# tsurumeso/vocal-remover

Measured on NVIDIA H100. Metric: seconds-of-audio/sec separated (n_fft=2048, hop=1024), higher is better.
Workload: dtype bf16x3 (split-bf16 operands hi+lo, 3 wgmma passes, fp32 accumulate); fft/lstm fp32

## Files before the change

### vocal-remover_b200/build.py

```python
import os
import subprocess
import sys
from concurrent.futures import ThreadPoolExecutor

HERE = os.path.dirname(os.path.abspath(__file__))
CSRC = os.path.join(HERE, 'csrc')
OBJ = os.path.join(HERE, 'build')
LIB = os.path.join(HERE, 'libvr_b200.so')
SOURCES = ['api.cu', 'engine.cu', 'conv_simt.cu', 'conv_tc.cu', 'conv_tc_rows.cu', 'conv_tc_halo.cu', 'elementwise.cu', 'lstm.cu', 'fft.cu', 'resample.cu', 'flac.cu', 'flac_encode.cu', 'bsseval.cu', 'wiener.cu']
NVCC = os.environ.get('NVCC', '/usr/local/cuda/bin/nvcc')
FLAGS = ['-gencode', 'arch=compute_90a,code=sm_90a', '-O3', '-lineinfo', '-std=c++17',
         '-Xcompiler', '-fPIC', '-Xcompiler', '-fvisibility=hidden', '--expt-relaxed-constexpr']


def _newest_header():
    hs = [os.path.join(CSRC, f) for f in os.listdir(CSRC) if f.endswith(('.h', '.cuh'))]
    hs.append(os.path.join(HERE, '..', 'include', 'vr_b200.h'))
    return max(os.path.getmtime(h) for h in hs)


def build(verbose=False, force=False):
    global OBJ, LIB
    extra = os.environ.get('VR_BUILD_FLAGS', '').split()
    if os.environ.get('VR_BUILD_TAG'):
        OBJ = os.path.join(HERE, 'build_' + os.environ['VR_BUILD_TAG'])
        LIB = os.path.join(HERE, 'libvr_b200_%s.so' % os.environ['VR_BUILD_TAG'])
    os.makedirs(OBJ, exist_ok=True)
    hdr = _newest_header()
    jobs = []
    for src in SOURCES:
        s = os.path.join(CSRC, src)
        o = os.path.join(OBJ, src.replace('.cu', '.o'))
        if force or not os.path.exists(o) or os.path.getmtime(o) < max(os.path.getmtime(s), hdr):
            jobs.append((s, o))

    def cc(job):
        s, o = job
        cmd = [NVCC] + FLAGS + extra + ['-c', s, '-o', o]
        if verbose:
            cmd += ['-Xptxas', '-v']
        r = subprocess.run(cmd, capture_output=True, text=True)
        if r.returncode != 0:
            raise RuntimeError('nvcc failed for %s:\n%s\n%s' % (s, r.stdout, r.stderr))
        return r.stderr

    with ThreadPoolExecutor(max_workers=min(8, max(1, len(jobs)))) as ex:
        logs = list(ex.map(cc, jobs))
    if verbose:
        for lg in logs:
            print(lg)
    objs = [os.path.join(OBJ, s.replace('.cu', '.o')) for s in SOURCES]
    if jobs or not os.path.exists(LIB):
        cmd = [NVCC, '-shared', '-o', LIB] + objs + ['-gencode', 'arch=compute_90a,code=sm_90a']
        r = subprocess.run(cmd, capture_output=True, text=True)
        if r.returncode != 0:
            raise RuntimeError('link failed:\n%s\n%s' % (r.stdout, r.stderr))
    return LIB


if __name__ == '__main__':
    print(build(verbose='-v' in sys.argv, force='-f' in sys.argv))
```

### vocal-remover_b200/csrc/api.cu

```cuda
#include <stdio.h>
#include <string.h>

#include <string>

#include "../../include/vr_b200.h"
#include "engine.h"
#include "kernels.h"
#include "tc_plan.h"

struct vr_ctx {
  vr::Engine* eng;
  std::string err;
};

static std::string g_create_err;

static int fail(vr_ctx* c, const std::string& m) {
  (c ? c->err : g_create_err) = m;
  return -1;
}
static void use_device(const vr_ctx* c) {
  if (c && c->eng) cudaSetDevice(c->eng->cfg().device);
}
static int done(vr_ctx* c, bool ok) {
// ... 339 lines not shown
  return 0;
}

int64_t vr_launch_count(const vr_ctx* ctx) { return ctx && ctx->eng ? ctx->eng->launches : 0; }

int vr_profile_enable(vr_ctx* ctx, int32_t on) {
  CHECK_CTX(ctx);
  ctx->eng->profile_enable(on != 0);
  return 0;
}

int vr_profile_read(vr_ctx* ctx, double* out6) {
  CHECK_CTX(ctx);
  return done(ctx, ctx->eng->profile_read(out6));
}

int vr_profile_dump(vr_ctx* ctx, char* text, int64_t cap, int64_t* needed) {
  CHECK_CTX(ctx);
  std::string t;
  if (!ctx->eng->profile_dump(t)) return done(ctx, false);
  if (needed) *needed = (int64_t)t.size() + 1;
  if (text && cap > 0) {
    const size_t n = t.size() < (size_t)cap - 1 ? t.size() : (size_t)cap - 1;
    memcpy(text, t.data(), n);
    text[n] = 0;
  }
  return 0;
}

int vr_debug_conv(vr_ctx* ctx, const float* x, int32_t N, int32_t Cin, int32_t H, int32_t W, const float* w,
                  const float* bias, int32_t Cout, int32_t k, int32_t stride, int32_t dil_h, int32_t dil_w, int32_t act,
                  int32_t use_tc, float* y, void* stream) {
  CHECK_CTX(ctx);
  return done(ctx, ctx->eng->debug_conv(x, N, Cin, H, W, w, bias, Cout, k, stride, dil_h, dil_w, act, use_tc, y,
                                        (cudaStream_t)stream));
}

int vr_debug_decoder(vr_ctx* ctx, const float* low, int32_t N, int32_t Cl, int32_t h, int32_t w, const float* skip,
                     int32_t Cs, const float* wgt, const float* bias, int32_t Cout, int32_t act, int32_t fused, float* y,
                     void* stream) {
  CHECK_CTX(ctx);
  return done(ctx, ctx->eng->debug_decoder(low, N, Cl, h, w, skip, Cs, wgt, bias, Cout, act, fused, y,
                                           (cudaStream_t)stream));
}

int vr_debug_tensor(vr_ctx* ctx, const char* name, int32_t n0, int32_t n, float* out, int64_t* shape4, void* stream) {
  CHECK_NET(ctx);
  if (!name || !shape4) return fail(ctx, "vr_debug_tensor: name and shape4 are required");
  return done(ctx, ctx->eng->debug_tensor(name, n0, n, out, shape4, (cudaStream_t)stream));
}

int vr_debug_set(int32_t key, int32_t value) {
  int* knob = key == 0 ? &vr::g_debug.trace : key == 2 ? &vr::g_debug.rows_wide : key == 3 ? &vr::g_debug.halo
            : key == 6 ? &vr::g_debug.kskip : key == 7 ? &vr::g_debug.crop_mask : nullptr;
  if (!knob) return -1;
  *knob = value;
  return 0;
}

int64_t vr_debug_trace(uint64_t* host_out, int64_t capacity) {
  return vr::tc_rows_read_trace((unsigned long long*)host_out, (long long)capacity);
}

}
```

### vocal-remover_b200/csrc/conv_tc.cu

```cuda
#include <cuda.h>
#include <stdio.h>

#include <map>
#include <tuple>

#include "engine.h"
#include "tc_common.cuh"
#include "tc_plan.h"

namespace vr {

static constexpr int kMaxStages = 8;
static constexpr int kConsumerWarps = 8;
static constexpr int kThreads = 32 * kConsumerWarps + 32;
static constexpr int kStaticSmem = 2048;

struct TcParams {
  int N, Ho, Wo, Wt, Ht, Nt, tiles_w, tiles_h, m_tiles, n_tiles;
  int stride, pad_h, pad_w, dil_h, dil_w, KW;
  int cchunks, total_sub, CinPadTC, Cout, act, stages;
  bf16* out_hi;
  bf16* out_lo;
  int64_t osn, osh;
  int osw;
// ... 103 lines not shown
        held.release(ring, lane);
        held.hold(ring);
        ring.advance();
      }
      wg_wait<0>();
      held.release_last(ring, lane);

      const int nt = tile % p.n_tiles;
      const int mt = tile / p.n_tiles;
      const int w0 = (mt % p.tiles_w) * p.Wt;
      const int h0 = ((mt / p.tiles_w) % p.tiles_h) * p.Ht;
      const int n0 = (mt / (p.tiles_w * p.tiles_h)) * p.Nt;
      const int c_lane = nt * BN + 2 * (lane & 3);
#pragma unroll
      for (int hr = 0; hr < 2; ++hr) {
        const int row = 64 * wg + 16 * (warp & 3) + (lane >> 2) + 8 * hr;
        const int dw = row % p.Wt;
        const int dh = (row / p.Wt) % p.Ht;
        const int n = n0 + row / (p.Wt * p.Ht);
        if (n >= p.N) continue;
        const int64_t obase = (int64_t)n * p.osn + (int64_t)(h0 + dh) * p.osh + (int64_t)(w0 + dw) * p.osw;
#pragma unroll
        for (int j = 0; j < BN / 8; ++j)
          epilogue_pair(acc[4 * j + 2 * hr], acc[4 * j + 2 * hr + 1], bias_s, c_lane + 8 * j, p.Cout, slope,
                        p.out_hi + obase, p.out_lo + obase);
      }
    }
  }
}

#define VR_TC_FOR_BN(X, KB) X(KB, 16) X(KB, 32) X(KB, 48) X(KB, 64) X(KB, 80) X(KB, 96) X(KB, 112) X(KB, 128)
#define VR_TC_FOR_ALL(X) VR_TC_FOR_BN(X, 64) VR_TC_FOR_BN(X, 32) VR_TC_FOR_BN(X, 16)


TcDebug g_debug;

static constexpr int kMaxDevices = 64;
const TcDevice& tc_device() {
  static TcDevice table[kMaxDevices];
  static TcDevice none;
  int dev = -1;
  if (cudaGetDevice(&dev) != cudaSuccess || dev < 0 || dev >= kMaxDevices) return none;
  TcDevice& d = table[dev];
  if (!d.ok) {
    if (cudaDeviceGetAttribute(&d.max_smem, cudaDevAttrMaxSharedMemoryPerBlockOptin, dev) != cudaSuccess ||
        cudaDeviceGetAttribute(&d.num_sms, cudaDevAttrMultiProcessorCount, dev) != cudaSuccess)
      return none;
#define VR_TC_SET_SMEM(KB, BN) \
  cudaFuncSetAttribute(conv_tc_kernel<KB, BN>, cudaFuncAttributeMaxDynamicSharedMemorySize, d.max_smem - kStaticSmem);
    VR_TC_FOR_ALL(VR_TC_SET_SMEM)
#undef VR_TC_SET_SMEM
    tc_rows_set_attributes(d.max_smem);
    tc_halo_set_attributes(d.max_smem);
    d.ok = true;
  }
  return d;
}

typedef CUresult (*EncodeTiledFn)(CUtensorMap*, CUtensorMapDataType, cuuint32_t, void*, const cuuint64_t*,
                                  const cuuint64_t*, const cuuint32_t*, const cuuint32_t*, CUtensorMapInterleave,
                                  CUtensorMapSwizzle, CUtensorMapL2promotion, CUtensorMapFloatOOBfill);
static EncodeTiledFn tc_encode_fn() {
  static EncodeTiledFn fn = nullptr;
  if (!fn) {
    void* p = nullptr;
    cudaDriverEntryPointQueryResult q;
    if (cudaGetDriverEntryPoint("cuTensorMapEncodeTiled", &p, cudaEnableDefault, &q) == cudaSuccess &&
        q == cudaDriverEntryPointSuccess)
      fn = (EncodeTiledFn)p;
  }
  return fn;
}

static CUtensorMapSwizzle swizzle_for(int KB) {
  return KB == 64 ? CU_TENSOR_MAP_SWIZZLE_128B : KB == 32 ? CU_TENSOR_MAP_SWIZZLE_64B : CU_TENSOR_MAP_SWIZZLE_32B;
}

static uint16_t tc_f2bf(float f) {
  uint32_t u;
  memcpy(&u, &f, 4);
  if ((u & 0x7fffffffu) > 0x7f800000u) return (uint16_t)((u >> 16) | 0x40);
  uint32_t r = 0x7fffu + ((u >> 16) & 1u);
  return (uint16_t)((u + r) >> 16);
}
static float tc_bf2f(uint16_t h) {
  uint32_t u = (uint32_t)h << 16;
  float f;
  memcpy(&f, &u, 4);
  return f;
}

struct TileGeom {
  int Wt, Ht, Nt;
  bool ok;
};
static TileGeom tile_geom(int Ho, int Wo) {
  TileGeom g{0, 0, 0, false};
  if (Wo <= 0 || Ho <= 0) return g;
  if (Wo >= 128) {
    if (Wo % 128) return g;
    g.Wt = 128; g.Ht = 1; g.Nt = 1;
  } else {
    if (128 % Wo) return g;
    g.Wt = Wo;
    g.Ht = 128 / Wo < Ho ? 128 / Wo : Ho;
    if (Ho % g.Ht) return g;
    if ((128 / Wo) % g.Ht) return g;
    g.Nt = 128 / (g.Wt * g.Ht);
  }
  g.ok = true;
  return g;
}

struct NTiling {
  int BN, n_tiles;
};
static NTiling n_tiling(const ConvLayer& L, bool rows, bool rows_wide) {
  const int cout16 = round_up(L.Cout, 16);
  if (rows) {
    const int BN = cout16 == 16 ? 16 : (rows_wide && cout16 % 64 == 0 ? 64 : 32);
    return {BN, ceil_div(cout16, BN)};
  }
  const int n_tiles = ceil_div(cout16, 128);
  return {round_up(ceil_div(cout16, n_tiles), 16), n_tiles};
}

TcKind tc_choose(const ConvLayer& L, int H, int W, bool rows_wide) {
  if (!(L.k == 1 || L.k == 3) || !(L.stride == 1 || L.stride == 2) || L.Cout < 4) return TC_NONE;
  const TileGeom g = tile_geom(H, W);
  if (!g.ok || g.Wt * L.stride > 256 || g.Ht * L.stride > 256) return TC_NONE;
  const bool k3s1 = L.k == 3 && L.stride == 1 && L.dil_h == 1 && L.dil_w == 1;
  const NTiling r = n_tiling(L, true, rows_wide), t = n_tiling(L, false, false);
  if (k3s1 && W % 128 == 0 && H % 8 == 0 && tc_rows_has(r.BN) && r.n_tiles * r.BN <= 256) return TC_ROWS;
  if (k3s1 && (W == 16 || W == 32 || W == 64) && H % (128 / W) == 0 && tc_halo_has(t.BN) &&
      t.n_tiles * t.BN <= 256 && g_debug.halo != 1)
    return TC_HALO;
  if (t.n_tiles * t.BN > 256) return TC_NONE;
  return TC_GENERIC;
}

template <class At>
static std::vector<uint16_t> split_bf16(const ConvLayer& L, const float* wp, int rows, int K, At at) {
  std::vector<uint16_t> planes((size_t)2 * rows * K, 0);
  const size_t lo = (size_t)rows * K;
  for (int co = 0; co < L.Cout; ++co)
    for (int t = 0; t < L.k * L.k; ++t)
      for (int ci = 0; ci < L.CinPad; ++ci) {
        const float w = wp[((size_t)t * L.CinPad + ci) * L.CoutPad + co];
        const uint16_t hi = tc_f2bf(w);
        const size_t i = at(co, t, ci);
        planes[i] = hi;
        planes[lo + i] = tc_f2bf(w - tc_bf2f(hi));
      }
  return planes;
}

static unsigned long long weight_group_mask(const ConvLayer& L, const float* wp, int CinPad) {
  if (CinPad / 8 > 64) return ~0ull;
  unsigned long long m = 0x3ull;
  for (int ci = 0; ci < L.CinPad; ++ci) {
    bool any = false;
    for (int t = 0; t < L.k * L.k && !any; ++t)
      for (int co = 0; co < L.Cout && !any; ++co) any = wp[((size_t)t * L.CinPad + ci) * L.CoutPad + co] != 0.f;
    if (any) m |= 1ull << (ci / 8);
  }
  return m;
}

static bool encode_weight_map(TcConv& tc, int rows, int K, int box_rows, std::string& err, const std::string& name) {
  cuuint64_t dims[3] = {(cuuint64_t)K, (cuuint64_t)rows, 2};
  cuuint64_t strides[2] = {(cuuint64_t)K * 2, (cuuint64_t)rows * K * 2};
  cuuint32_t box[3] = {(cuuint32_t)tc.KB, (cuuint32_t)box_rows, 2};
  cuuint32_t es[3] = {1, 1, 1};
  CUresult r = tc_encode_fn()(&tc.map_b, CU_TENSOR_MAP_DATA_TYPE_BFLOAT16, 3, tc.w_planes.get(), dims, strides, box, es,
                              CU_TENSOR_MAP_INTERLEAVE_NONE, swizzle_for(tc.KB), CU_TENSOR_MAP_L2_PROMOTION_L2_256B,
                              CU_TENSOR_MAP_FLOAT_OOB_FILL_NONE);
  if (r != CUDA_SUCCESS) {
    err = "cuTensorMapEncodeTiled(weights) failed for " + name + " code " + std::to_string((int)r);
    return false;
  }
  return true;
}

const CUtensorMap* tc_activation_map(TcConv& tc, const ActView& v, int bw, int bh, int bn, int es, std::string& err,
                                     const std::string& name) {
  const ViewKey key = std::make_tuple((const void*)v.hi, (const void*)v.lo, v.N, v.H, v.W, v.C, bw, bh, bn);
  auto it = tc.map_a.find(key);
  if (it != tc.map_a.end()) return &it->second;
  const int64_t plane = (const char*)v.lo - (const char*)v.hi;
  if (v.sw % 8 || v.sh % 8 || v.sn % 8 || (reinterpret_cast<uintptr_t>(v.hi) & 15) || plane <= 0 || plane % 16) {
    err = "internal: the input of " + name + " is not 16-byte aligned or its lo plane does not follow its hi plane";
    return nullptr;
  }
  cuuint64_t dims[5] = {(cuuint64_t)v.C, (cuuint64_t)v.W, (cuuint64_t)v.H, (cuuint64_t)v.N, 2};
  cuuint64_t strides[4] = {(cuuint64_t)v.sw * 2, (cuuint64_t)v.sh * 2, (cuuint64_t)v.sn * 2, (cuuint64_t)plane};
  cuuint32_t box[5] = {(cuuint32_t)tc.KB, (cuuint32_t)bw, (cuuint32_t)bh, (cuuint32_t)bn, 2};
  cuuint32_t estr[5] = {1, (cuuint32_t)es, (cuuint32_t)es, 1, 1};
  CUtensorMap m;
  CUresult r = tc_encode_fn()(&m, CU_TENSOR_MAP_DATA_TYPE_BFLOAT16, 5, (void*)v.hi, dims, strides, box, estr,
                              CU_TENSOR_MAP_INTERLEAVE_NONE, swizzle_for(tc.KB), CU_TENSOR_MAP_L2_PROMOTION_L2_256B,
                              CU_TENSOR_MAP_FLOAT_OOB_FILL_NONE);
  if (r != CUDA_SUCCESS) {
    err = "cuTensorMapEncodeTiled(activations) failed for " + name + " code " + std::to_string((int)r);
    return nullptr;
  }
  return &tc.map_a.emplace(key, m).first->second;
}

bool tc_prepare(ConvLayer& L, const float* w, const float* b, int H, int W, bool rows_wide, std::string& err) {
  const TcKind kind = tc_choose(L, H, W, rows_wide);
  if (kind == TC_NONE) return true;
  if (!tc_encode_fn()) {
    err = "cuTensorMapEncodeTiled is not available from the driver";
    return false;
  }
  auto tc = std::make_shared<TcConv>();
  tc->kind = kind;
  tc->H = H; tc->W = W;
  const NTiling nt = n_tiling(L, kind == TC_ROWS, rows_wide);
  const int BN = nt.BN, cin16 = round_up(L.CinPad, 16);
  tc->BN = BN; tc->n_tiles = nt.n_tiles;
  tc->KB = kind != TC_GENERIC ? 32 : cin16 % 64 == 0 ? 64 : cin16 % 32 == 0 ? 32 : 16;
  const int CinPad = round_up(L.CinPad, tc->KB);
  tc->CinPad = CinPad;
  tc->chunks = CinPad / tc->KB;
  tc->kmask = weight_group_mask(L, w, CinPad);
  const int rows = nt.n_tiles * BN;
  std::vector<uint16_t> planes;
  int brows, K;
  if (kind == TC_ROWS) {
    brows = 3 * rows;
    K = 3 * CinPad;
    planes = split_bf16(L, w, brows, K, [&](int co, int t, int ci) {
      return (size_t)(co / BN * 3 * BN + (2 - t / 3) * BN + co % BN) * K + (size_t)(t % 3) * CinPad + ci;
    });
  } else {
    brows = rows;
    K = L.k * L.k * CinPad;
    planes = split_bf16(L, w, brows, K, [&](int co, int t, int ci) { return (size_t)co * K + (size_t)t * CinPad + ci; });
  }
  std::vector<float> bias((size_t)rows, 0.f);
  for (int co = 0; co < L.Cout; ++co) bias[(size_t)co] = b[co];
  if (tc->w_planes.alloc(planes.size() * 2) != cudaSuccess || tc->bias.alloc(bias.size() * 4) != cudaSuccess) {
    err = "cudaMalloc failed while packing tensor-core weights for " + L.name;
    return false;
  }
  if (!upload(tc->w_planes.get(), planes.data(), planes.size() * 2, err) ||
      !upload(tc->bias.get(), bias.data(), bias.size() * 4, err) ||
      !encode_weight_map(*tc, brows, K, kind == TC_ROWS ? 3 * BN : BN, err, L.name))
    return false;
  L.tc = tc;
  return true;
}

cudaError_t tc_launch(const ConvLayer& L, const ActView& in, const ActView& out, cudaStream_t s, std::string& err,
                      const ConvFusion& f) {
  TcConv& tc = *L.tc;
  if (out.H != tc.H || out.W != tc.W || (in.H - 1) / L.stride + 1 != out.H || (in.W - 1) / L.stride + 1 != out.W) {
    err = "internal: " + L.name + " is launched on maps of another size than it was prepared for";
    return cudaErrorInvalidValue;
  }
  if (tc.kind == TC_ROWS) return tc_rows_launch(L, tc, in, out, s, err, f);
  if (!f.empty()) {
    err = "tc_launch: fused work is only implemented in the row-streaming kernel";
    return cudaErrorInvalidValue;
  }
  if (tc.kind == TC_HALO) return tc_halo_launch(L, tc, in, out, s, err);
  const TileGeom g = tile_geom(out.H, out.W);
  const CUtensorMap* map_a = tc_activation_map(tc, in, g.Wt * L.stride, g.Ht * L.stride, g.Nt, L.stride, err, L.name);
  if (!map_a) return cudaErrorInvalidValue;
  const int SUBS = 64 / tc.KB;
  TcParams p;
  p.N = out.N; p.Ho = out.H; p.Wo = out.W;
  p.Wt = g.Wt; p.Ht = g.Ht; p.Nt = g.Nt;
  p.tiles_w = out.W / g.Wt; p.tiles_h = out.H / g.Ht;
  p.m_tiles = p.tiles_w * p.tiles_h * ceil_div(out.N, g.Nt);
  p.n_tiles = tc.n_tiles;
  p.stride = L.stride; p.dil_h = L.dil_h; p.dil_w = L.dil_w;
  p.pad_h = L.dil_h * (L.k / 2); p.pad_w = L.dil_w * (L.k / 2);
  p.KW = L.k;
  p.cchunks = tc.chunks; p.total_sub = L.k * L.k * tc.chunks;
  p.CinPadTC = tc.CinPad; p.Cout = L.Cout; p.act = L.act;
  const int stage_bytes = SUBS * (2 * 128 * tc.KB * 2 + 2 * tc.BN * tc.KB * 2);
  const TcDevice& dv = tc_device();
  if (!dv.ok) {
    err = "tc_launch: cannot query the current device";
    return cudaErrorInvalidValue;
  }
  const int dyn = dv.max_smem - kStaticSmem;
  p.stages = (dyn - 1024) / stage_bytes;
  if (p.stages > kMaxStages) p.stages = kMaxStages;
  if (p.stages < 2) {
    err = "tc_launch: shared memory too small for two pipeline stages";
    return cudaErrorInvalidValue;
  }
  p.out_hi = out.hi; p.out_lo = out.lo;
  p.osn = out.sn; p.osh = out.sh; p.osw = out.sw;
  p.bias = tc.bias.get();
  const int total_tiles = p.m_tiles * p.n_tiles;
  const int grid = total_tiles < dv.num_sms ? total_tiles : dv.num_sms;
#define VR_TC_LAUNCH(KB_, BN_)                                                       \
  if (tc.KB == KB_ && tc.BN == BN_) {                                                \
    conv_tc_kernel<KB_, BN_><<<grid, kThreads, dyn, s>>>(*map_a, tc.map_b, p);       \
    return cudaGetLastError();                                                       \
  }
  VR_TC_FOR_ALL(VR_TC_LAUNCH)
#undef VR_TC_LAUNCH
  err = "tc_launch: no kernel instantiation for this channel tile";
  return cudaErrorInvalidValue;
}

}
```

### vocal-remover_b200/csrc/conv_tc_halo.cu

```cuda
#include <stdio.h>

#include "engine.h"
#include "tc_common.cuh"
#include "tc_plan.h"

namespace vr {

static constexpr int kConsumerWarps = 8;
static constexpr int kProducerWarps = 4;
static constexpr int kThreads = 32 * (kConsumerWarps + kProducerWarps);
static constexpr int kLaunchRegs = 168;
static constexpr int kConsumerRegs = 232;
static constexpr int kProducerRegs = 40;
static_assert(kConsumerWarps * kConsumerRegs + kProducerWarps * kProducerRegs <=
                  (kConsumerWarps + kProducerWarps) * kLaunchRegs,
              "setmaxnreg.inc would wait forever for registers the block does not own");
static constexpr int kStaticSmem = 2048;
static constexpr int kMaxHSlots = 4;
static constexpr int kMaxWStages = 18;
static constexpr uint32_t kKB = 32;
static constexpr uint32_t kRowB = kKB * 2;

template <int BN>
struct HaloGeom {
// ... 149 lines not shown
              (int64_t)n * p.osn + (int64_t)(h0 + (px >> p.lw)) * p.osh + (int64_t)(px & (p.W - 1)) * p.osw;
          const float* v = acc + b * (BN / 2) + 2 * hr;
#pragma unroll
          for (int j = 0; j < BN / 8; ++j)
            epilogue_pair(v[4 * j], v[4 * j + 1], bias_s, c_lane + 8 * j, p.Cout, slope, p.out_hi + obase,
                          p.out_lo + obase);
        }
      }
    }
  }
}

#define VR_HALO_FOR_MB(X, BN) X(BN, 1) X(BN, 2)
#define VR_HALO_FOR_ALL(X) \
  VR_HALO_FOR_MB(X, 16) VR_HALO_FOR_MB(X, 32) VR_HALO_FOR_MB(X, 48) VR_HALO_FOR_MB(X, 64) VR_HALO_FOR_MB(X, 96) \
  VR_HALO_FOR_MB(X, 128)

bool tc_halo_has(int BN) {
#define VR_HALO_HAS(BN_, MB_) if (BN == BN_) return true;
  VR_HALO_FOR_ALL(VR_HALO_HAS)
#undef VR_HALO_HAS
  return false;
}

cudaError_t tc_halo_launch(const ConvLayer& L, TcConv& tc, const ActView& in, const ActView& out, cudaStream_t s,
                           std::string& err) {
  const TcDevice& dv = tc_device();
  if (!dv.ok) {
    err = "tc_halo_launch: cannot query the current device";
    return cudaErrorInvalidValue;
  }
  const int ht1 = 128 / out.W;
  const bool mb2_tiles = out.H % (2 * ht1) == 0;
  const int tiles1 = out.N * (out.H / ht1) * tc.n_tiles;
  const int waves1 = ceil_div(tiles1, dv.num_sms), waves2 = ceil_div(tiles1 / 2, dv.num_sms);
  int MB = mb2_tiles && 19 * waves2 <= 10 * waves1 ? 2 : 1;
  if (g_debug.halo == 2) MB = 1;
  if (g_debug.halo == 3 && mb2_tiles) MB = 2;
  HaloParams p;
  p.N = out.N; p.H = out.H; p.W = out.W;
  p.lw = out.W == 16 ? 4 : out.W == 32 ? 5 : 6;
  p.Ht = MB * ht1;
  p.Wb = round_up(out.W + 2, 8);
  p.tiles_h = out.H / p.Ht;
  p.n_tiles = tc.n_tiles;
  p.total_tiles = out.N * p.tiles_h * p.n_tiles;
  p.chunks = tc.chunks; p.CinPadH = tc.CinPad; p.Cout = L.Cout; p.act = L.act;
  p.hplane = (uint32_t)((p.Ht + 2) * p.Wb) * kRowB;
  p.hslot = 2 * p.hplane;
  p.kmask = g_debug.kskip == 1 ? tc.kmask : ~0ull;
  p.out_hi = out.hi; p.out_lo = out.lo;
  p.osn = out.sn; p.osh = out.sh; p.osw = out.sw;
  p.bias = tc.bias.get();
  const CUtensorMap* map_a = tc_activation_map(tc, in, p.Wb, p.Ht + 2, 1, 1, err, L.name);
  if (!map_a) return cudaErrorInvalidValue;
  const int w_stage = tc.BN * 2 * (int)kRowB;
  const int dyn = dv.max_smem - kStaticSmem;
  const int avail = dyn - 1024;
  p.n_hslots = (avail - 9 * w_stage) / (int)p.hslot;
  if (p.n_hslots > kMaxHSlots) p.n_hslots = kMaxHSlots;
  if (p.n_hslots < 2) p.n_hslots = 2;
  p.n_wstages = (avail - p.n_hslots * (int)p.hslot) / w_stage;
  if (p.n_wstages > kMaxWStages) p.n_wstages = kMaxWStages;
  if (p.n_wstages < 2) {
    err = "tc_halo_launch: shared memory too small for two halo slots and two weight stages";
    return cudaErrorInvalidValue;
  }
  const int grid = p.total_tiles < dv.num_sms ? p.total_tiles : dv.num_sms;
#define VR_HALO_LAUNCH(BN_, MB_)                                                        \
  if (tc.BN == BN_ && MB == MB_) {                                                      \
    conv_tc_halo_kernel<BN_, MB_><<<grid, kThreads, dyn, s>>>(*map_a, tc.map_b, p);     \
    return cudaGetLastError();                                                          \
  }
  VR_HALO_FOR_ALL(VR_HALO_LAUNCH)
#undef VR_HALO_LAUNCH
  err = "tc_halo_launch: no kernel instantiation for this channel tile";
  return cudaErrorInvalidValue;
}


void tc_halo_set_attributes(int max_smem) {
#define VR_HALO_SET(BN_, MB_) \
  cudaFuncSetAttribute(conv_tc_halo_kernel<BN_, MB_>, cudaFuncAttributeMaxDynamicSharedMemorySize, max_smem - kStaticSmem);
  VR_HALO_FOR_ALL(VR_HALO_SET)
#undef VR_HALO_SET
}

}
```

### vocal-remover_b200/csrc/conv_tc_rows.cu

```cuda
#include <stdio.h>

#include "engine.h"
#include "tc_common.cuh"
#include "tc_plan.h"

namespace vr {

static constexpr int kInterpWarps = 10;
static constexpr int kConsumerWarps = 8;
static constexpr int kTmaWarp = kConsumerWarps;
static constexpr int kInterpWarp0 = kConsumerWarps + 1;
__host__ __device__ constexpr int rows_per_tile(int BN) { return BN == 64 ? 2 : BN == 32 ? 4 : 8; }
static constexpr int kUpProducerWarps = 12;
static constexpr int kUpConsumerRegs = 128;
static constexpr int kUpProducerRegs = 72;
static constexpr int kUpLaunchRegs = 96;
static_assert(kConsumerWarps * kUpConsumerRegs + kUpProducerWarps * kUpProducerRegs <=
                  (kConsumerWarps + kUpProducerWarps) * kUpLaunchRegs,
              "setmaxnreg.inc would wait forever for registers the block does not own");
__host__ __device__ constexpr int rows_threads(bool up) { return 32 * (kConsumerWarps + (up ? kUpProducerWarps : 1)); }
static constexpr int kRowPx = 130;
static constexpr int kBoxPx = 136;
static constexpr int kMaxASlots = 8;
static constexpr int kStaticSmem = 3072;
// ... 403 lines not shown
                bf16x8 oh, ol;
                split8(y, oh, ol);
                *reinterpret_cast<uint4*>(slot + e_off[k]) = oh;
                *reinterpret_cast<uint4*>(slot + kAPlane + e_off[k]) = ol;
              }
              if (z_off >= 0) {
                *reinterpret_cast<uint4*>(slot + z_off) = make_uint4(0, 0, 0, 0);
                *reinterpret_cast<uint4*>(slot + kAPlane + z_off) = make_uint4(0, 0, 0, 0);
              }
              warp_arrive(a_up.full(), lane);
              fetch();
              if (tr && lane == 0 && tn < kTraceEvents) {
                g_rows_trace[(2 * kTraceEvents + tn) * 3 + 0] = t0;
                g_rows_trace[(2 * kTraceEvents + tn) * 3 + 1] = t2 - t1;
                g_rows_trace[(2 * kTraceEvents + tn) * 3 + 2] = clock64();
              }
              ++tn;
              a_up.advance();
            }
          }
        }
      }
      }
  }
}

#define VR_ROWS_FOR_ALL(X) X(16, true) X(16, false) X(32, true) X(32, false) X(64, true) X(64, false)

static int rows_b_bytes(int BN) {
#define VR_ROWS_B(BN_, UP_) if (BN == BN_) return (int)(2 * RowsGeom<BN_>::kBBuf);
  VR_ROWS_FOR_ALL(VR_ROWS_B)
#undef VR_ROWS_B
  return 0;
}

bool tc_rows_has(int BN) { return rows_b_bytes(BN) > 0; }

cudaError_t tc_rows_launch(const ConvLayer& L, TcConv& tc, const ActView& in, const ActView& out, cudaStream_t s,
                           std::string& err, const ConvFusion& f) {
  const ActView* up_src = f.up;
  if (up_src && (!tc.fuses_upsample(up_src->C) || up_src->H * 2 != in.H || up_src->W * 2 != in.W || up_src->sw % 8)) {
    err = "tc_rows_launch: fused upsample needs a half-resolution source of 32k channels";
    return cudaErrorInvalidValue;
  }
  if (up_src && up_src->C + in.C > tc.CinPad) {
    err = "tc_rows_launch: with a fused upsample the input must hold only the channels after the up-sampled ones";
    return cudaErrorInvalidValue;
  }
  const ActView* last = f.last_chunk;
  if (last && (last->H != in.H || last->W != in.W || last->N != in.N || last->C > tc.KB)) {
    err = "tc_rows_launch: the last-chunk tensor must match the input geometry and fit one chunk";
    return cudaErrorInvalidValue;
  }
  const CUtensorMap* map_a = tc_activation_map(tc, in, kBoxPx, 1, 1, 1, err, L.name);
  const CUtensorMap* map_l = last ? tc_activation_map(tc, *last, kBoxPx, 1, 1, 1, err, L.name) : map_a;
  if (!map_a || !map_l) return cudaErrorInvalidValue;
  if (f.mask && !tc.fuses_mask(L.Cout, f.mask->offset, up_src != nullptr)) {
    err = "tc_rows_launch: the fused output layer needs a fused upsample, one N tile of Cout <= 32 channels and a "
          "kept width that is a multiple of 128";
    return cudaErrorInvalidValue;
  }
  const int col0 = f.mask ? f.mask->offset : 0;
  RowsParams p;
  p.N = out.N; p.H = out.H; p.W = out.W;
  const bool up = up_src != nullptr;
  p.col0 = col0;
  p.tiles_w = (out.W - 2 * col0) / 128; p.tiles_h = out.H / rows_per_tile(tc.BN); p.n_tiles = tc.n_tiles;
  p.total_tiles = p.tiles_w * p.tiles_h * out.N * tc.n_tiles;
  p.chunks = tc.chunks; p.CinPadR = tc.CinPad; p.Cout = L.Cout; p.act = L.act;
  p.out_hi = out.hi; p.out_lo = out.lo;
  p.osn = out.sn; p.osh = out.sh; p.osw = out.sw;
  p.bias = tc.bias.get();
  p.up_chunks = 0; p.xH = p.xW = 0;
  p.x_hi = p.x_lo = nullptr; p.xsn = p.xsh = 0; p.xsw = 0;
  p.trace = g_debug.trace == 1 ? 1 : 0;
  p.up_sh = p.up_sw = 0.f;
  p.dot_w = f.dot_w; p.dot_out = f.dot_w ? f.dot_out : nullptr;
  p.mask = f.mask ? *f.mask : MaskOutParams{};
  p.a_c_off = 0;
  p.l_chunk = last ? tc.chunks - 1 : -1;
  p.kmask = g_debug.kskip == 1 ? tc.kmask : ~0ull;
  if (up_src) {
    p.a_c_off = -up_src->C;
    p.up_chunks = up_src->C / 32;
    p.xH = up_src->H; p.xW = up_src->W;
    p.x_hi = up_src->hi; p.x_lo = up_src->lo;
    p.xsn = up_src->sn; p.xsh = up_src->sh; p.xsw = up_src->sw;
    if ((reinterpret_cast<uintptr_t>(up_src->hi) | reinterpret_cast<uintptr_t>(up_src->lo)) & 15) {
      err = "tc_rows_launch: upsample source planes must be 16-byte aligned";
      return cudaErrorInvalidValue;
    }
    p.up_sh = in.H > 1 ? (float)(up_src->H - 1) / (float)(in.H - 1) : 0.f;
    p.up_sw = in.W > 1 ? (float)(up_src->W - 1) / (float)(in.W - 1) : 0.f;
  }
  const TcDevice& dv = tc_device();
  if (!dv.ok) {
    err = "tc_rows_launch: cannot query the current device";
    return cudaErrorInvalidValue;
  }
  const int b_bytes = rows_b_bytes(tc.BN);
  p.n_aslots = (dv.max_smem - kStaticSmem - 1024 - b_bytes) / (int)kASlot;
  if (p.n_aslots > kMaxASlots) p.n_aslots = kMaxASlots;
  if (p.n_aslots < (p.up_chunks > 0 ? 4 : 2)) {
    err = "tc_rows_launch: shared memory too small";
    return cudaErrorInvalidValue;
  }
  p.n_uslots = p.up_chunks > 0 ? p.n_aslots - p.n_aslots / 2 : 0;
  if (p.up_chunks > 0 && p.n_aslots - p.n_uslots < 2) p.n_uslots = p.n_aslots - 2;
// ... 33 lines not shown
```

### vocal-remover_b200/csrc/tc_plan.h

```cpp
#pragma once
#include <cuda.h>

#include <map>
#include <tuple>

#include "engine.h"

namespace vr {

enum TcKind {
  TC_NONE,
  TC_GENERIC,
  TC_ROWS,
  TC_HALO,
};

typedef std::tuple<const void*, const void*, int, int, int, int, int, int, int> ViewKey;

struct TcConv {
  TcKind kind = TC_NONE;
  int H = 0, W = 0;
  int KB = 0, CinPad = 0, chunks = 0, BN = 0, n_tiles = 0;
  unsigned long long kmask = ~0ull;
  DevPtr<bf16> w_planes;
  DevPtr<float> bias;
  CUtensorMap map_b;
  std::map<ViewKey, CUtensorMap> map_a;
  bool fuses_upsample(int up_C) const { return kind == TC_ROWS && up_C % 32 == 0 && up_C <= CinPad; }
  bool fuses_dot() const { return kind == TC_ROWS; }
  bool fuses_mask(int Cout, int offset, bool up) const {
    const int kept = W - 2 * offset;
    return kind == TC_ROWS && up && n_tiles == 1 && BN <= 32 && BN == Cout && offset >= 0 && kept > 0 &&
           kept % 128 == 0;
  }
};

TcKind tc_choose(const ConvLayer& L, int H, int W, bool rows_wide);
const CUtensorMap* tc_activation_map(TcConv& tc, const ActView& v, int bw, int bh, int bn, int es, std::string& err,
                                     const std::string& name);

cudaError_t tc_rows_launch(const ConvLayer& L, TcConv& tc, const ActView& in, const ActView& out, cudaStream_t s,
                           std::string& err, const ConvFusion& f);
void tc_rows_set_attributes(int max_smem);
bool tc_rows_has(int BN);
int tc_rows_read_trace(unsigned long long* out, long long capacity);

cudaError_t tc_halo_launch(const ConvLayer& L, TcConv& tc, const ActView& in, const ActView& out, cudaStream_t s,
                           std::string& err);
void tc_halo_set_attributes(int max_smem);
bool tc_halo_has(int BN);

struct TcDevice {
  bool ok = false;
  int num_sms = 0, max_smem = 0;
};
const TcDevice& tc_device();

struct TcDebug {
  int trace = 0;
  int rows_wide = 0;
  int halo = 0;
  int kskip = 1;
  int crop_mask = 1;
};
extern TcDebug g_debug;

}
```

Before: 2873.

## Add halo-reuse tensor-core kernel for narrow 3x3 stride-2 convolutions

Adds a dedicated warp-specialized wgmma kernel for 3x3 stride-2 convolutions with few input channels. It loads one even/odd-column-split halo tile per channel chunk through TMA and reuses it across all nine taps, where the generic kernel refetches a strided box for each tap. The kernel streams weights per tap, rebalances registers with setmaxnreg, and picks one or two M blocks per tile from a wave-count heuristic. In exchange it adds many template instantiations and a new selection path that generic layers may now take, with layout and swizzle math that must exactly match the TMA boxes.

New measurement: 2907 (median of 6 runs). +1.2%, better.

```diff
diff --git a/vocal-remover_b200/build.py b/vocal-remover_b200/build.py
--- a/vocal-remover_b200/build.py
+++ b/vocal-remover_b200/build.py
@@ -7,7 +7,7 @@
 CSRC = os.path.join(HERE, 'csrc')
 OBJ = os.path.join(HERE, 'build')
 LIB = os.path.join(HERE, 'libvr_b200.so')
-SOURCES = ['api.cu', 'engine.cu', 'conv_simt.cu', 'conv_tc.cu', 'conv_tc_rows.cu', 'conv_tc_halo.cu', 'elementwise.cu', 'lstm.cu', 'fft.cu', 'resample.cu', 'flac.cu', 'flac_encode.cu', 'bsseval.cu', 'wiener.cu']
+SOURCES = ['api.cu', 'engine.cu', 'conv_simt.cu', 'conv_tc.cu', 'conv_tc_rows.cu', 'conv_tc_halo.cu', 'conv_tc_strided.cu', 'elementwise.cu', 'lstm.cu', 'fft.cu', 'resample.cu', 'flac.cu', 'flac_encode.cu', 'bsseval.cu', 'wiener.cu']
 NVCC = os.environ.get('NVCC', '/usr/local/cuda/bin/nvcc')
 FLAGS = ['-gencode', 'arch=compute_90a,code=sm_90a', '-O3', '-lineinfo', '-std=c++17',
          '-Xcompiler', '-fPIC', '-Xcompiler', '-fvisibility=hidden', '--expt-relaxed-constexpr']
diff --git a/vocal-remover_b200/csrc/api.cu b/vocal-remover_b200/csrc/api.cu
--- a/vocal-remover_b200/csrc/api.cu
+++ b/vocal-remover_b200/csrc/api.cu
@@ -415,7 +415,8 @@
 
 int vr_debug_set(int32_t key, int32_t value) {
   int* knob = key == 0 ? &vr::g_debug.trace : key == 2 ? &vr::g_debug.rows_wide : key == 3 ? &vr::g_debug.halo
-            : key == 6 ? &vr::g_debug.kskip : key == 7 ? &vr::g_debug.crop_mask : nullptr;
+            : key == 6 ? &vr::g_debug.kskip : key == 7 ? &vr::g_debug.crop_mask : key == 8 ? &vr::g_debug.strided
+            : nullptr;
   if (!knob) return -1;
   *knob = value;
   return 0;
diff --git a/vocal-remover_b200/csrc/conv_tc.cu b/vocal-remover_b200/csrc/conv_tc.cu
--- a/vocal-remover_b200/csrc/conv_tc.cu
+++ b/vocal-remover_b200/csrc/conv_tc.cu
@@ -179,6 +179,7 @@
 #undef VR_TC_SET_SMEM
     tc_rows_set_attributes(d.max_smem);
     tc_halo_set_attributes(d.max_smem);
+    tc_strided_set_attributes(d.max_smem);
     d.ok = true;
   }
   return d;
@@ -263,6 +264,12 @@
       t.n_tiles * t.BN <= 256 && g_debug.halo != 1)
     return TC_HALO;
   if (t.n_tiles * t.BN > 256) return TC_NONE;
+  const bool k3s2 = L.k == 3 && L.stride == 2 && L.dil_h == 1 && L.dil_w == 1;
+  const int cin16 = round_up(L.CinPad, 16);
+  const bool narrow = cin16 == 16 || (cin16 == 32 && W >= 32) || g_debug.strided >= 2;
+  if (k3s2 && narrow && (W == 16 || W == 32 || W == 64 || W == 128) && H % (128 / tc_strided_wt(W)) == 0 &&
+      tc_strided_has(t.BN) && g_debug.strided != 1)
+    return TC_STRIDED;
   return TC_GENERIC;
 }
 
@@ -309,8 +316,8 @@
   return true;
 }
 
-const CUtensorMap* tc_activation_map(TcConv& tc, const ActView& v, int bw, int bh, int bn, int es, std::string& err,
-                                     const std::string& name) {
+const CUtensorMap* tc_activation_map(TcConv& tc, const ActView& v, int bw, int bh, int bn, int es_w, int es_h,
+                                     std::string& err, const std::string& name) {
   const ViewKey key = std::make_tuple((const void*)v.hi, (const void*)v.lo, v.N, v.H, v.W, v.C, bw, bh, bn);
   auto it = tc.map_a.find(key);
   if (it != tc.map_a.end()) return &it->second;
@@ -322,7 +329,7 @@
   cuuint64_t dims[5] = {(cuuint64_t)v.C, (cuuint64_t)v.W, (cuuint64_t)v.H, (cuuint64_t)v.N, 2};
   cuuint64_t strides[4] = {(cuuint64_t)v.sw * 2, (cuuint64_t)v.sh * 2, (cuuint64_t)v.sn * 2, (cuuint64_t)plane};
   cuuint32_t box[5] = {(cuuint32_t)tc.KB, (cuuint32_t)bw, (cuuint32_t)bh, (cuuint32_t)bn, 2};
-  cuuint32_t estr[5] = {1, (cuuint32_t)es, (cuuint32_t)es, 1, 1};
+  cuuint32_t estr[5] = {1, (cuuint32_t)es_w, (cuuint32_t)es_h, 1, 1};
   CUtensorMap m;
   CUresult r = tc_encode_fn()(&m, CU_TENSOR_MAP_DATA_TYPE_BFLOAT16, 5, (void*)v.hi, dims, strides, box, estr,
                               CU_TENSOR_MAP_INTERLEAVE_NONE, swizzle_for(tc.KB), CU_TENSOR_MAP_L2_PROMOTION_L2_256B,
@@ -347,7 +354,7 @@
   const NTiling nt = n_tiling(L, kind == TC_ROWS, rows_wide);
   const int BN = nt.BN, cin16 = round_up(L.CinPad, 16);
   tc->BN = BN; tc->n_tiles = nt.n_tiles;
-  tc->KB = kind != TC_GENERIC ? 32 : cin16 % 64 == 0 ? 64 : cin16 % 32 == 0 ? 32 : 16;
+  tc->KB = kind == TC_STRIDED ? tc_strided_kb(L.CinPad, W) : kind != TC_GENERIC ? 32 : cin16 % 64 == 0 ? 64 : cin16 % 32 == 0 ? 32 : 16;
   const int CinPad = round_up(L.CinPad, tc->KB);
   tc->CinPad = CinPad;
   tc->chunks = CinPad / tc->KB;
@@ -393,8 +400,10 @@
     return cudaErrorInvalidValue;
   }
   if (tc.kind == TC_HALO) return tc_halo_launch(L, tc, in, out, s, err);
+  if (tc.kind == TC_STRIDED) return tc_strided_launch(L, tc, in, out, s, err);
   const TileGeom g = tile_geom(out.H, out.W);
-  const CUtensorMap* map_a = tc_activation_map(tc, in, g.Wt * L.stride, g.Ht * L.stride, g.Nt, L.stride, err, L.name);
+  const CUtensorMap* map_a = tc_activation_map(tc, in, g.Wt * L.stride, g.Ht * L.stride, g.Nt, L.stride, L.stride, err,
+                                                     L.name);
   if (!map_a) return cudaErrorInvalidValue;
   const int SUBS = 64 / tc.KB;
   TcParams p;
diff --git a/vocal-remover_b200/csrc/conv_tc_halo.cu b/vocal-remover_b200/csrc/conv_tc_halo.cu
--- a/vocal-remover_b200/csrc/conv_tc_halo.cu
+++ b/vocal-remover_b200/csrc/conv_tc_halo.cu
@@ -225,7 +225,7 @@
   p.out_hi = out.hi; p.out_lo = out.lo;
   p.osn = out.sn; p.osh = out.sh; p.osw = out.sw;
   p.bias = tc.bias.get();
-  const CUtensorMap* map_a = tc_activation_map(tc, in, p.Wb, p.Ht + 2, 1, 1, err, L.name);
+  const CUtensorMap* map_a = tc_activation_map(tc, in, p.Wb, p.Ht + 2, 1, 1, 1, err, L.name);
   if (!map_a) return cudaErrorInvalidValue;
   const int w_stage = tc.BN * 2 * (int)kRowB;
   const int dyn = dv.max_smem - kStaticSmem;
diff --git a/vocal-remover_b200/csrc/conv_tc_rows.cu b/vocal-remover_b200/csrc/conv_tc_rows.cu
--- a/vocal-remover_b200/csrc/conv_tc_rows.cu
+++ b/vocal-remover_b200/csrc/conv_tc_rows.cu
@@ -479,8 +479,8 @@
     err = "tc_rows_launch: the last-chunk tensor must match the input geometry and fit one chunk";
     return cudaErrorInvalidValue;
   }
-  const CUtensorMap* map_a = tc_activation_map(tc, in, kBoxPx, 1, 1, 1, err, L.name);
-  const CUtensorMap* map_l = last ? tc_activation_map(tc, *last, kBoxPx, 1, 1, 1, err, L.name) : map_a;
+  const CUtensorMap* map_a = tc_activation_map(tc, in, kBoxPx, 1, 1, 1, 1, err, L.name);
+  const CUtensorMap* map_l = last ? tc_activation_map(tc, *last, kBoxPx, 1, 1, 1, 1, err, L.name) : map_a;
   if (!map_a || !map_l) return cudaErrorInvalidValue;
   if (f.mask && !tc.fuses_mask(L.Cout, f.mask->offset, up_src != nullptr)) {
     err = "tc_rows_launch: the fused output layer needs a fused upsample, one N tile of Cout <= 32 channels and a "
diff --git a/vocal-remover_b200/csrc/conv_tc_strided.cu b/vocal-remover_b200/csrc/conv_tc_strided.cu
--- /dev/null
+++ b/vocal-remover_b200/csrc/conv_tc_strided.cu
@@ -0,0 +1,291 @@
+#include <stdio.h>
+
+#include "engine.h"
+#include "tc_common.cuh"
+#include "tc_plan.h"
+
+namespace vr {
+
+static constexpr int kConsumerWarps = 8;
+static constexpr int kProducerWarps = 4;
+static constexpr int kThreads = 32 * (kConsumerWarps + kProducerWarps);
+static constexpr int kLaunchRegs = 168;
+static constexpr int kConsumerRegs = 232;
+static constexpr int kProducerRegs = 40;
+static_assert(kConsumerWarps * kConsumerRegs + kProducerWarps * kProducerRegs <=
+                  (kConsumerWarps + kProducerWarps) * kLaunchRegs,
+              "setmaxnreg.inc would wait forever for registers the block does not own");
+static constexpr int kStaticSmem = 2048;
+static constexpr int kMaxHSlots = 4;
+static constexpr int kMaxWStages = 18;
+
+template <int KB, int BN>
+struct StridedGeom {
+  static constexpr uint32_t kRowB = KB * 2;
+  static constexpr int kSteps = KB / 16;
+  static constexpr uint32_t kBPlane = BN * kRowB;
+  static constexpr uint32_t kWStage = 2 * kBPlane;
+  static constexpr uint32_t kLayout = KB == 16 ? 3u : 2u;
+};
+
+struct StridedParams {
+  int lw, Wb, tiles_w, tiles_h, n_tiles, total_tiles;
+  int chunks, CinPadS, Cout, act;
+  int n_hslots, n_wstages;
+  uint32_t hplane, hpar, hslot;
+  unsigned long long kmask;
+  bf16* out_hi;
+  bf16* out_lo;
+  int64_t osn, osh;
+  int osw;
+  const float* bias;
+};
+
+struct StridedTile {
+  int nt, n, h0, w0;
+};
+__device__ __forceinline__ StridedTile strided_tile(const StridedParams& p, int tile, int Ht) {
+  StridedTile t;
+  t.nt = tile % p.n_tiles;
+  int mt = tile / p.n_tiles;
+  t.w0 = (mt % p.tiles_w) << p.lw;
+  mt /= p.tiles_w;
+  t.h0 = (mt % p.tiles_h) * Ht;
+  t.n = mt / p.tiles_h;
+  return t;
+}
+
+template <int KB>
+__device__ __forceinline__ uint32_t chunk_bits(unsigned long long kmask, int cc) {
+  constexpr int kBits = KB / 8;
+  const int sh = cc * kBits;
+  return sh + kBits <= 64 ? (uint32_t)(kmask >> sh) & ((1u << kBits) - 1u) : 1u;
+}
+
+struct StridedConsumer {
+  MbarRing h, w;
+  HeldSlot held_w;
+};
+
+template <int KB, int BN, int MB>
+__device__ __forceinline__ void consume_strided(StridedConsumer& st, const StridedParams& p, float* acc,
+                                                uint32_t (&fr)[3][MB * 8], const uint32_t* q0, uint32_t h_base,
+                                                uint32_t w_base, uint32_t dhi, int lane) {
+  typedef StridedGeom<KB, BN> G;
+  st.h.wait_full();
+  const uint32_t slot = h_base + (uint32_t)st.h.slot * p.hslot;
+#pragma unroll
+  for (int t = 0; t < 9; ++t) {
+    const int kh = t / 3, kw = t % 3;
+    const uint32_t box = slot + (kw == 1 ? p.hpar : 0u);
+#pragma unroll
+    for (int ks = 0; ks < G::kSteps; ++ks) {
+      uint32_t* f = fr[(G::kSteps * t + ks) % 3];
+#pragma unroll
+      for (int b = 0; b < MB; ++b) {
+        const uint32_t q = q0[b] + (uint32_t)(kh * p.Wb + (kw == 2 ? 1 : 0));
+        const uint32_t sw = KB == 16 ? (q >> 2) & 1u : (q >> 1) & 3u;
+        const uint32_t a = box + q * G::kRowB + ((((uint32_t)(2 * ks) + ((uint32_t)lane >> 4)) ^ sw) << 4);
+        ldsm_x4(f + 8 * b, a);
+        ldsm_x4(f + 8 * b + 4, a + p.hplane);
+      }
+      if (ks == 0) st.w.wait_full();
+      const uint32_t b_hi = desc_lo(w_base + (uint32_t)st.w.slot * G::kWStage) + (uint32_t)(ks * 32 >> 4);
+      wg_fence();
+#pragma unroll
+      for (int b = 0; b < MB; ++b)
+        wgmma_split3_rs<BN>(acc + b * (BN / 2), f + 8 * b, f + 8 * b + 4, b_hi, b_hi + (G::kBPlane >> 4), dhi);
+      wg_commit();
+      if (t == 8 && ks == G::kSteps - 1) warp_arrive(st.h.empty(), lane);
+      wg_wait<1>();
+      st.held_w.release(st.w, lane);
+    }
+    st.held_w.hold(st.w);
+    st.w.advance();
+  }
+  st.h.advance();
+}
+
+template <int KB, int BN, int MB>
+__global__ void __launch_bounds__(kThreads, 1)
+    conv_tc_strided_kernel(const __grid_constant__ CUtensorMap tmA, const __grid_constant__ CUtensorMap tmB,
+                           const StridedParams p) {
+  typedef StridedGeom<KB, BN> G;
+  extern __shared__ uint8_t smem_raw[];
+  __shared__ __align__(8) uint64_t bar_hfull[kMaxHSlots];
+  __shared__ __align__(8) uint64_t bar_hempty[kMaxHSlots];
+  __shared__ __align__(8) uint64_t bar_wfull[kMaxWStages];
+  __shared__ __align__(8) uint64_t bar_wempty[kMaxWStages];
+  __shared__ float bias_s[256];
+
+  const int warp = __shfl_sync(0xffffffffu, (int)threadIdx.x >> 5, 0);
+  const int lane = threadIdx.x & 31;
+  const int Ht = (128 * MB) >> p.lw;
+  const uint32_t smem_base = (smem_u32(smem_raw) + 1023u) & ~1023u;
+  const uint32_t h_base = smem_base;
+  const uint32_t w_base = smem_base + (uint32_t)p.n_hslots * p.hslot;
+  MbarRing hring(smem_u32(&bar_hfull[0]), smem_u32(&bar_hempty[0]), 0, p.n_hslots);
+  MbarRing wring(smem_u32(&bar_wfull[0]), smem_u32(&bar_wempty[0]), 0, p.n_wstages);
+
+  if (warp == kConsumerWarps && lane == 0) {
+    tma_prefetch(&tmA);
+    tma_prefetch(&tmB);
+    hring.init(1, kConsumerWarps);
+    wring.init(1, kConsumerWarps);
+    asm volatile("fence.mbarrier_init.release.cluster;" ::: "memory");
+  }
+  for (int i = threadIdx.x; i < p.n_tiles * BN; i += blockDim.x) bias_s[i] = __ldg(p.bias + i);
+  __syncthreads();
+
+  if (warp >= kConsumerWarps) {
+    setmaxnreg_dec<kProducerRegs>();
+    if (warp == kConsumerWarps && elect_one_sync()) {
+      for (int tile = blockIdx.x; tile < p.total_tiles; tile += gridDim.x) {
+        const StridedTile tt = strided_tile(p, tile, Ht);
+        for (int cc = 0; cc < p.chunks; ++cc) {
+          if (!chunk_bits<KB>(p.kmask, cc)) continue;
+          hring.wait_empty();
+          const uint32_t dst = h_base + (uint32_t)hring.slot * p.hslot;
+          mbar_expect_tx(hring.full(), p.hslot);
+          tma_load_5d(dst, &tmA, cc * KB, 2 * tt.w0 - 1, 2 * tt.h0 - 1, tt.n, 0, hring.full());
+          tma_load_5d(dst + p.hpar, &tmA, cc * KB, 2 * tt.w0, 2 * tt.h0 - 1, tt.n, 0, hring.full());
+          hring.advance();
+          for (int t = 0; t < 9; ++t) {
+            wring.wait_empty();
+            mbar_expect_tx(wring.full(), G::kWStage);
+            tma_load_3d(w_base + (uint32_t)wring.slot * G::kWStage, &tmB, t * p.CinPadS + cc * KB,
+                        tt.nt * BN, 0, wring.full());
+            wring.advance();
+          }
+        }
+      }
+    }
+    __syncwarp();
+  } else {
+    setmaxnreg_inc<kConsumerRegs>();
+    const int wg = warp >> 2;
+    const float slope = act_slope(p.act);
+    const uint32_t dhi = desc_hi(8 * G::kRowB, G::kLayout);
+    const int wmask = (1 << p.lw) - 1;
+    uint32_t q0[MB];
+#pragma unroll
+    for (int b = 0; b < MB; ++b) {
+      const int px = 64 * (MB * wg + b) + 16 * (warp & 3) + (lane & 15);
+      q0[b] = (uint32_t)(2 * (px >> p.lw) * p.Wb + (px & wmask));
+    }
+    StridedConsumer st{hring, wring};
+    float acc[MB * BN / 2];
+    uint32_t fr[3][MB * 8];
+    for (int tile = blockIdx.x; tile < p.total_tiles; tile += gridDim.x) {
+#pragma unroll
+      for (int i = 0; i < MB * BN / 2; ++i) acc[i] = 0.f;
+      for (int cc = 0; cc < p.chunks; ++cc) {
+        if (!chunk_bits<KB>(p.kmask, cc)) continue;
+        consume_strided<KB, BN, MB>(st, p, acc, fr, q0, h_base, w_base, dhi, lane);
+      }
+      wg_wait<0>();
+      st.held_w.release_last(st.w, lane);
+
+      const StridedTile tt = strided_tile(p, tile, Ht);
+      const int c_lane = tt.nt * BN + 2 * (lane & 3);
+#pragma unroll
+      for (int b = 0; b < MB; ++b) {
+#pragma unroll
+        for (int hr = 0; hr < 2; ++hr) {
+          const int px = 64 * (MB * wg + b) + 16 * (warp & 3) + (lane >> 2) + 8 * hr;
+          const int64_t obase = (int64_t)tt.n * p.osn + (int64_t)(tt.h0 + (px >> p.lw)) * p.osh +
+                                (int64_t)(tt.w0 + (px & wmask)) * p.osw;
+          const float* v = acc + b * (BN / 2) + 2 * hr;
+#pragma unroll
+          for (int j = 0; j < BN / 8; ++j)
+            epilogue_pair(v[4 * j], v[4 * j + 1], bias_s, c_lane + 8 * j, p.Cout, slope, p.out_hi + obase,
+                          p.out_lo + obase);
+        }
+      }
+    }
+  }
+}
+
+#define VR_STRIDED_FOR_BN(X, KB, MB) X(KB, 16, MB) X(KB, 32, MB) X(KB, 48, MB) X(KB, 64, MB) X(KB, 96, MB) X(KB, 128, MB)
+#define VR_STRIDED_FOR_ALL(X) VR_STRIDED_FOR_BN(X, 16, 1) VR_STRIDED_FOR_BN(X, 16, 2) VR_STRIDED_FOR_BN(X, 32, 1)
+
+bool tc_strided_has(int BN) {
+#define VR_STRIDED_HAS(KB_, BN_, MB_) if (BN == BN_) return true;
+  VR_STRIDED_FOR_ALL(VR_STRIDED_HAS)
+#undef VR_STRIDED_HAS
+  return false;
+}
+
+int tc_strided_wt(int W) { return W < 64 ? W : 64; }
+
+int tc_strided_kb(int CinPad, int W) { return round_up(CinPad, 16) == 32 && W >= 32 ? 32 : 16; }
+
+cudaError_t tc_strided_launch(const ConvLayer& L, TcConv& tc, const ActView& in, const ActView& out, cudaStream_t s,
+                              std::string& err) {
+  const TcDevice& dv = tc_device();
+  if (!dv.ok) {
+    err = "tc_strided_launch: cannot query the current device";
+    return cudaErrorInvalidValue;
+  }
+  const int Wt = tc_strided_wt(out.W);
+  const int tiles_w = out.W / Wt;
+  const int ht1 = 128 / Wt;
+  const bool mb2_tiles = out.H % (2 * ht1) == 0;
+  const int tiles1 = out.N * (out.H / ht1) * tiles_w * tc.n_tiles;
+  const int waves1 = ceil_div(tiles1, dv.num_sms), waves2 = ceil_div(tiles1 / 2, dv.num_sms);
+  int MB = mb2_tiles && 19 * waves2 <= 10 * waves1 ? 2 : 1;
+  if (g_debug.strided == 2) MB = 1;
+  if (g_debug.strided == 3 && mb2_tiles) MB = 2;
+  if (tc.KB == 32) MB = 1;
+  const int row_b = tc.KB * 2;
+  const int Ht = MB * ht1, Hb = 2 * Ht + 1;
+  StridedParams p;
+  p.lw = Wt == 16 ? 4 : Wt == 32 ? 5 : 6;
+  p.Wb = round_up(Wt + 1, 8);
+  p.tiles_w = tiles_w;
+  p.tiles_h = out.H / Ht;
+  p.n_tiles = tc.n_tiles;
+  p.total_tiles = out.N * p.tiles_h * p.tiles_w * p.n_tiles;
+  p.chunks = tc.chunks; p.CinPadS = tc.CinPad; p.Cout = L.Cout; p.act = L.act;
+  p.hplane = (uint32_t)(Hb * p.Wb * row_b);
+  p.hpar = 2 * p.hplane;
+  p.hslot = 2 * p.hpar;
+  p.kmask = g_debug.kskip == 1 ? tc.kmask : ~0ull;
+  p.out_hi = out.hi; p.out_lo = out.lo;
+  p.osn = out.sn; p.osh = out.sh; p.osw = out.sw;
+  p.bias = tc.bias.get();
+  const CUtensorMap* map_a = tc_activation_map(tc, in, 2 * p.Wb, Hb, 1, 2, 1, err, L.name);
+  if (!map_a) return cudaErrorInvalidValue;
+  const int w_stage = tc.BN * 2 * row_b;
+  const int dyn = dv.max_smem - kStaticSmem;
+  const int avail = dyn - 1024;
+  p.n_hslots = (avail - 9 * w_stage) / (int)p.hslot;
+  if (p.n_hslots > kMaxHSlots) p.n_hslots = kMaxHSlots;
+  if (p.n_hslots < 2) p.n_hslots = 2;
+  p.n_wstages = (avail - p.n_hslots * (int)p.hslot) / w_stage;
+  if (p.n_wstages > kMaxWStages) p.n_wstages = kMaxWStages;
+  if (p.n_wstages < 2) {
+    err = "tc_strided_launch: shared memory too small for two input slots and two weight stages";
+    return cudaErrorInvalidValue;
+  }
+  const int grid = p.total_tiles < dv.num_sms ? p.total_tiles : dv.num_sms;
+#define VR_STRIDED_LAUNCH(KB_, BN_, MB_)                                                      \
+  if (tc.KB == KB_ && tc.BN == BN_ && MB == MB_) {                                            \
+    conv_tc_strided_kernel<KB_, BN_, MB_><<<grid, kThreads, dyn, s>>>(*map_a, tc.map_b, p);   \
+    return cudaGetLastError();                                                                \
+  }
+  VR_STRIDED_FOR_ALL(VR_STRIDED_LAUNCH)
+#undef VR_STRIDED_LAUNCH
+  err = "tc_strided_launch: no kernel instantiation for this channel tile";
+  return cudaErrorInvalidValue;
+}
+
+void tc_strided_set_attributes(int max_smem) {
+#define VR_STRIDED_SET(KB_, BN_, MB_)                                                                   \
+  cudaFuncSetAttribute(conv_tc_strided_kernel<KB_, BN_, MB_>, cudaFuncAttributeMaxDynamicSharedMemorySize, \
+                       max_smem - kStaticSmem);
+  VR_STRIDED_FOR_ALL(VR_STRIDED_SET)
+#undef VR_STRIDED_SET
+}
+
+}
diff --git a/vocal-remover_b200/csrc/tc_plan.h b/vocal-remover_b200/csrc/tc_plan.h
--- a/vocal-remover_b200/csrc/tc_plan.h
+++ b/vocal-remover_b200/csrc/tc_plan.h
@@ -13,6 +13,7 @@
   TC_GENERIC,
   TC_ROWS,
   TC_HALO,
+  TC_STRIDED,
 };
 
 typedef std::tuple<const void*, const void*, int, int, int, int, int, int, int> ViewKey;
@@ -36,8 +37,8 @@
 };
 
 TcKind tc_choose(const ConvLayer& L, int H, int W, bool rows_wide);
-const CUtensorMap* tc_activation_map(TcConv& tc, const ActView& v, int bw, int bh, int bn, int es, std::string& err,
-                                     const std::string& name);
+const CUtensorMap* tc_activation_map(TcConv& tc, const ActView& v, int bw, int bh, int bn, int es_w, int es_h,
+                                     std::string& err, const std::string& name);
 
 cudaError_t tc_rows_launch(const ConvLayer& L, TcConv& tc, const ActView& in, const ActView& out, cudaStream_t s,
                            std::string& err, const ConvFusion& f);
@@ -49,6 +50,13 @@
                            std::string& err);
 void tc_halo_set_attributes(int max_smem);
 bool tc_halo_has(int BN);
+
+cudaError_t tc_strided_launch(const ConvLayer& L, TcConv& tc, const ActView& in, const ActView& out, cudaStream_t s,
+                              std::string& err);
+void tc_strided_set_attributes(int max_smem);
+bool tc_strided_has(int BN);
+int tc_strided_wt(int W);
+int tc_strided_kb(int CinPad, int W);
 
 struct TcDevice {
   bool ok = false;
@@ -62,6 +70,7 @@
   int halo = 0;
   int kskip = 1;
   int crop_mask = 1;
+  int strided = 0;
 };
 extern TcDebug g_debug;
 
```
